# ada-shen/Interpret_quality

Hardware: AMD Instinct MI355X
Metric: coalitions/sec (masked forward passes/sec), PointNet 1024-pt ModelNet10 (higher is better)
Workload: dtype f32; 1 GPU; PointNet ModelNet10-style Shapley, 32 regions x 1000 permutations per cloud (33000 coalitions per step per GPU), BASELINE configs[1]; permutations sampled and masked on the device inside the timed step; num_points=1024, num_regions=32, permutations=1000, parallelism=clouds sharded over 1 GPU(s), one all_gather_into_tensor of the logits per step

## Files before the change

include/iq.h:

```cpp
#ifndef IQ_H_
#define IQ_H_

#include <stddef.h>
#include <stdint.h>

#ifdef __cplusplus
extern "C" {
#endif

typedef void* iq_stream_t;

enum {
    IQ_OK = 0,
    IQ_EINVAL = -1,
    IQ_ELAUNCH = -2,
    IQ_EWORKSPACE = -3,
    IQ_EUNSUPPORTED = -4
};

#define IQ_MAX_REGIONS 64
#define IQ_MAX_POINTS 4096
#define IQ_NUM_FEAT 1024
#define IQ_MAX_EXACT_PLAYERS 24
#define IQ_MAX_WIDE_REGIONS 1024

#define IQ_ABI_VERSION 111
int iq_version(void);
const char* iq_last_error(void);


int iq_mask_shapley(const float* cloud , const int32_t* region_id ,
                    const int32_t* orders , const float* center , float* out,
                    int N, int R, int bs, int channel_first, iq_stream_t stream);

int iq_mask_interaction(const float* cloud , const int32_t* region_id ,
                        const int32_t* pairs , const uint64_t* ctx_mask ,
                        const float* center , float* out ,
                        int N, int R, int nb, iq_stream_t stream);

int iq_mask_coalitions(const float* cloud , const int32_t* region_id ,
                       const uint64_t* keep , const float* center , float* out,
                       int N, int B, int channel_first, iq_stream_t stream);

int iq_check_index_range(const int32_t* idx, size_t count, int lo, int hi, uint32_t* scratch ,
                         iq_stream_t stream);


int iq_sample_permutations(uint32_t* mt_state , int32_t* orders , int S, int R, iq_stream_t stream);

size_t iq_sample_workspace_bytes(int S, int R);
int iq_sample_permutations_ws(uint32_t* mt_state , int32_t* orders , int S, int R, void* workspace,
                              size_t workspace_bytes, iq_stream_t stream);

int iq_prefix_keep_masks(const int32_t* orders , uint64_t* keep , int S, int R, iq_stream_t stream);

int iq_context_keep_masks(const int32_t* pairs , const int32_t* contexts , uint64_t* keep ,
                          int P, int C, int m, iq_stream_t stream);


int iq_reward(const float* logits , int label, int modified, float* v ,
              int B, int C, iq_stream_t stream);

int iq_shapley_accum(const float* v , const int32_t* orders ,
                     double* sv_rows, double* phi_sum, const int32_t* snap_counts, int n_snap,
                     double* snaps, int R, int S, iq_stream_t stream);

int iq_interaction_reduce(const float* v , float* out , int n, iq_stream_t stream);


int iq_region_assign(const float* cloud , const int32_t* fps_idx ,
                     int32_t* region_id , int N, int R, iq_stream_t stream);

int iq_fps(const float* xyz, int32_t* idx, int B, int N, int S, iq_stream_t stream);

typedef struct iq_smoothness_params {
    double step;
    double enum_step;
    double var_threshold;
    double dist_threshold;
// ... 234 lines not shown
```

include/iq_debug.h:

```cpp
#ifndef IQ_DEBUG_H_
#define IQ_DEBUG_H_

#include "iq.h"

#ifdef __cplusplus
extern "C" {
#endif

int iq_profile_enable(int on);
int iq_profile_read_work(int slot, double* total_ms, int* launches, double* total_work);
int iq_set_tuning(int key, int value);
int iq_profile_read(int slot, double* total_ms, int* launches);

int iq_debug_mfma_sustained(double seconds, float* scratch , size_t scratch_floats, double* tflops ,
                            double* clock_ghz , iq_stream_t stream);
int iq_debug_mfma_sustained_shape(int shape, double seconds, float* scratch , size_t scratch_floats, double* tflops ,
                                  double* clock_ghz , iq_stream_t stream);

#ifdef __cplusplus
}
#endif
#endif
```

interpret_quality_amd/_lib.py:

```python
import ctypes
import os

from . import build as _build

_HERE = os.path.dirname(os.path.abspath(__file__))

c_f32p = ctypes.c_void_p
c_ptr = ctypes.c_void_p


class IqError(RuntimeError):
    pass


class DenseLayer(ctypes.Structure):
    _fields_ = [("w", ctypes.c_void_p), ("b", ctypes.c_void_p), ("cin", ctypes.c_int32), ("cout", ctypes.c_int32),
                ("w_bf3", ctypes.c_void_p)]


class PointNetWeights(ctypes.Structure):
    _fields_ = [
        ("stn_in", ctypes.c_void_p),
        ("stn_c2", DenseLayer), ("stn_c3", DenseLayer), ("stn_fc1", DenseLayer), ("stn_fc2", DenseLayer),
        ("stn_fc3", DenseLayer),
# ... 78 lines not shown
                                    _I, _I, _I, _I, _I, _P]),
    "iq_pointnet_coalitions_crt": (_I, [ctypes.POINTER(PointNetWeights), _P, _P, _P, _P, _P, _P, _P, _P, _P, _SZ,
                                        _I, _I, _I, _I, _I, _P]),
    "iq_pointnet_flops_per_coalition": (ctypes.c_double, [_I]),
    "iq_ball_query": (_I, [_P, _P, ctypes.c_float, _I, _P, _I, _I, _I, _P]),
    "iq_pointnet2_workspace_bytes": (_SZ, [_I]),
    "iq_pointnet2_forward": (_I, [ctypes.POINTER(PointNet2Weights), _P, _P, _P, _SZ, _I, _I, _P]),
    "iq_pointnet2_coalitions_workspace_bytes": (_SZ, [_I, _I, _I]),
    "iq_pointnet2_coalitions": (_I, [ctypes.POINTER(PointNet2Weights), _P, _P, _P, _P, _P, _P, _P, _SZ, _I, _I, _I, _P]),
    "iq_knn": (_I, [_P, _P, _P, _SZ, _I, _I, _I, _I, _P]),
    "iq_dgcnn_workspace_bytes": (_SZ, [_I, _I]),
    "iq_dgcnn_forward": (_I, [ctypes.POINTER(DgcnnWeights), _P, _P, _P, _SZ, _I, _I, _I, _P]),
    "iq_dgcnn_coalitions": (_I, [ctypes.POINTER(DgcnnWeights), _P, _P, _P, _P, _P, _P, _P, _SZ, _I, _I, _I, _I, _P]),
    "iq_pointconv_workspace_bytes": (_SZ, [_I, _I]),
    "iq_pointconv_forward": (_I, [ctypes.POINTER(PointConvWeights), _P, _P, _P, _SZ, _I, _I, _P]),
    "iq_pointconv_coalitions_workspace_bytes": (_SZ, [_I, _I, _I]),
    "iq_pointconv_coalitions": (_I, [ctypes.POINTER(PointConvWeights), _P, _P, _P, _P, _P, _P, _P, _SZ, _I, _I, _I, _P]),
    "iq_pointconv_tables_bytes": (_SZ, [_I, _I]),
    "iq_pointconv_coalitions_cached": (_I, [ctypes.POINTER(PointConvWeights), _P, _P, _P, _P, _P, _P, _P, _SZ, _I, _I, _I,
                                          ctypes.POINTER(ctypes.c_int), _P]),
    "iq_index_points": (_I, [_P, _P, _P, _I, _I, _I, _I, _P]),
    "iq_group_points": (_I, [_P, _P, _P, _P, _P, _I, _I, _I, _I, _I, _I, _P]),
    "iq_edgeconv_gather": (_I, [_P, _P, _P, _I, _I, _I, _I, _I, _P]),
    "iq_knn_point": (_I, [_P, _P, _I, _P, _P, _SZ, _I, _I, _I, _P]),
    "iq_sort_neighbours": (_I, [_P, _P, _P, _I, _I, _I, _I, _I, _P]),
    "iq_density": (_I, [_P, ctypes.c_double, _P, _I, _I, _P]),
    "iq_enum_keep_masks": (_I, [_P, ctypes.c_uint64, _SZ, _P, _I, ctypes.c_uint64, _P]),
    "iq_exact_scratch_bytes": (_SZ, [_I, _I]),
    "iq_exact_shapley": (_I, [_P, _I, _P, _P, _SZ, _P]),
    "iq_exact_interactions": (_I, [_P, _I, _P, _I, _P, _P, _SZ, _P]),
    "iq_moebius": (_I, [_P, _I, _P, _P]),
    "iq_prefix_keep_masks_wide": (_I, [_P, _P, _I, _I, _P]),
    "iq_context_keep_masks_wide": (_I, [_P, _P, _P, _I, _I, _I, _I, _P]),
    "iq_mask_coalitions_wide": (_I, [_P, _P, _P, _P, _P, _I, _I, _I, _I, _P]),
    "iq_region_assign_wide": (_I, [_P, _P, _P, _I, _I, _P]),
    "iq_shapley_accum_wide": (_I, [_P, _P, _P, _P, _P, _I, _P, _I, _I, _P]),
    "iq_pointnet_wide_workspace_bytes": (_SZ, [_I, _I, _I, _I]),
    "iq_pointnet_coalitions_wide": (_I, [ctypes.POINTER(PointNetWeights), _P, _P, _P, _P, _P, _P, _P, _P, _SZ,
                                         _I, _I, _I, _I, _I, _P]),
    "iq_pointnet_prefix_coalitions_wide": (_I, [ctypes.POINTER(PointNetWeights), _P, _P, _P, _P, _P, _P, _P, _P, _SZ,
                                                _I, _I, _I, _I, _P]),
    "iq_dgcnn_coalitions_wide": (_I, [ctypes.POINTER(DgcnnWeights), _P, _P, _P, _P, _P, _P, _P, _SZ, _I, _I, _I, _I, _I, _P]),
    "iq_pointnet2_coalitions_wide": (_I, [ctypes.POINTER(PointNet2Weights), _P, _P, _P, _P, _P, _P, _P, _SZ, _I, _I, _I, _I, _P]),
    "iq_pointconv_coalitions_wide": (_I, [ctypes.POINTER(PointConvWeights), _P, _P, _P, _P, _P, _P, _P, _SZ, _I, _I, _I, _I, _P]),
    "iq_pointconv_coalitions_cached_wide": (_I, [ctypes.POINTER(PointConvWeights), _P, _P, _P, _P, _P, _P, _P, _SZ, _I, _I, _I,
                                               ctypes.POINTER(ctypes.c_int), _I, _P]),
    "iq_profile_enable": (_I, [_I]),
    "iq_set_tuning": (_I, [_I, _I]),
    "iq_profile_read_work": (_I, [_I, ctypes.POINTER(ctypes.c_double), ctypes.POINTER(ctypes.c_int), ctypes.POINTER(ctypes.c_double)]),
    "iq_profile_read": (_I, [_I, ctypes.POINTER(ctypes.c_double), ctypes.POINTER(ctypes.c_int)]),
    "iq_debug_mfma_sustained": (_I, [ctypes.c_double, _P, _SZ, ctypes.POINTER(ctypes.c_double), ctypes.POINTER(ctypes.c_double), _P]),
    "iq_debug_mfma_sustained_shape": (_I, [_I, ctypes.c_double, _P, _SZ, ctypes.POINTER(ctypes.c_double),
                                           ctypes.POINTER(ctypes.c_double), _P]),
}

_lib = None
ABI_VERSION = 111


def lib_path():
    return os.environ.get("IQ_LIBPATH") or _build.LIBPATH


def load():
    global _lib
    if _lib is not None:
        return _lib
    import torch
    path = lib_path()
    if not os.path.exists(path):
        raise IqError("libiq_hip.so not found at %s - run `python -m interpret_quality_amd.build` "
                      "(there is no CPU or PyTorch fallback for the HIP path)" % path)
    lib = ctypes.CDLL(path)
    for name, (res, args) in SIGNATURES.items():
        fn = getattr(lib, name)
        fn.restype = res
        fn.argtypes = args
    if lib.iq_version() != ABI_VERSION:
        raise IqError("%s reports ABI version %d, these bindings are written for %d - rebuild it (python -m interpret_quality_amd.build "
                      "--force)" % (path, lib.iq_version(), ABI_VERSION))
    _lib = lib
    return lib


def check(rc, what):
    if rc != 0:
        msg = load().iq_last_error()
        raise IqError("%s failed (%d): %s" % (what, rc, msg.decode() if msg else ""))
```

interpret_quality_amd/csrc/iq_pointnet.hip:

```cpp
#include <algorithm>

#include "iq_pointnet_chain.h"

namespace {

template <int MAXR>
__device__ __forceinline__ void pn_prepare_body(const int32_t* __restrict__ region_id, uint16_t* __restrict__ sorted_pts,
                                                int32_t* __restrict__ roff, int N, int R) {
    constexpr int kWaves = kThreads / 64;
    __shared__ int16_t rid[kMaxN];
    __shared__ int cnt[kWaves][MAXR + 1];
    const int cloud = blockIdx.x, tid = threadIdx.x, wave = tid >> 6, lane = tid & 63;
    for (int r = tid; r <= R; r += kThreads)
        for (int w = 0; w < kWaves; ++w) cnt[w][r] = 0;
    for (int p = tid; p < N; p += kThreads) {
        const int r = region_id[(size_t)cloud * N + p];
        rid[p] = (int16_t)((unsigned)r < (unsigned)R ? r : R);
    }
    __syncthreads();
    const int per = (N + kThreads - 1) / kThreads * 64;
    const int begin = min(wave * per, N), end = min(begin + per, N);
    for (int p = begin + lane; p < end; p += 64) atomicAdd(&cnt[wave][rid[p]], 1);
    __syncthreads();
    if (wave == 0) {
// ... 317 lines not shown
    const int item = blockIdx.x * blockDim.x + threadIdx.x;
    int bin = 0, pos = 0;
    if (item < B) {
        bin = bin_of[item];
        pos = atomicAdd(&lh[bin], 1);
    }
    __syncthreads();
    if (threadIdx.x < kBins && lh[threadIdx.x]) base[threadIdx.x] = atomicAdd(&cursor[threadIdx.x], lh[threadIdx.x]);
    __syncthreads();
    if (item < B) order[base[bin] + pos] = item;
}

constexpr int kOrderThreads = 1024, kOrderPer = 4, kOrderFusedMax = kOrderThreads * kOrderPer;

__global__ __launch_bounds__(kOrderThreads) void pn_order_fused_kernel(const int32_t* __restrict__ nrows_all,
                                                                       int32_t* __restrict__ order, int B) {
    __shared__ int lh[kBins];
    const int tid = threadIdx.x, lane = tid & 63;
    if (tid < kBins) lh[tid] = 0;
    __syncthreads();
    int bin[kOrderPer], pos[kOrderPer];
#pragma unroll
    for (int j = 0; j < kOrderPer; ++j) {
        const int item = tid + j * kOrderThreads;
        if (item < B) {
            const int rows = nrows_all[item] & 0xffff;
            bin[j] = kBins - 1 - min(kBins - 1, (rows + kMC - 1) / kMC);
            pos[j] = atomicAdd(&lh[bin[j]], 1);
        }
    }
    __syncthreads();
    if (tid < 64) {
        int carry = 0;
        for (int b0 = 0; b0 < kBins; b0 += 64) {
            const int b = b0 + lane, c = b < kBins ? lh[b] : 0;
            int inc = c;
#pragma unroll
            for (int off = 1; off < 64; off <<= 1) {
                const int t = __shfl_up(inc, off);
                if (lane >= off) inc += t;
            }
            if (b < kBins) lh[b] = carry + inc - c;
            carry += __shfl(inc, 63);
        }
    }
    __syncthreads();
#pragma unroll
    for (int j = 0; j < kOrderPer; ++j) {
        const int item = tid + j * kOrderThreads;
        if (item < B) order[lh[bin[j]] + pos[j]] = item;
    }
}

constexpr int kDupRepOff = kBins;
static_assert(iq::align_up((kBins + 2) * sizeof(int32_t), 256) == iq::align_up(kBins * sizeof(int32_t), 256), "room behind hist");

__global__ __launch_bounds__(kOrderThreads) void pn_dup_rep_kernel(const int32_t* __restrict__ nrows_all, int32_t* __restrict__ rep,
                                                                   int B, int N) {
    __shared__ int first[2];
    if (threadIdx.x < 2) first[threadIdx.x] = B;
    __syncthreads();
    for (int item = threadIdx.x; item < B; item += kOrderThreads) {
        const int kind = dup_kind(nrows_all[item], N);
        if (kind >= 0) atomicMin(&first[kind], item);
    }
    __syncthreads();
    if (threadIdx.x < 2) rep[threadIdx.x] = first[threadIdx.x];
}

__global__ __launch_bounds__(kThreads) void pn_dup_copy_kernel(const int32_t* __restrict__ nrows_all, const int32_t* __restrict__ rep,
                                                               float* __restrict__ out, int32_t* __restrict__ argrow, int N) {
    const int item = blockIdx.x;
    const int kind = dup_kind(nrows_all[item], N);
    if (kind < 0) return;
    const int src = rep[kind];
    if (src == item) return;
    static_assert(kFeat == 4 * kThreads, "one float4 per thread");
    reinterpret_cast<f32x4*>(out + (size_t)item * kFeat)[threadIdx.x] = reinterpret_cast<const f32x4*>(out + (size_t)src * kFeat)[threadIdx.x];
    if (argrow) {
        const int4 v = reinterpret_cast<const int4*>(argrow + (size_t)src * kFeat)[threadIdx.x];
        reinterpret_cast<int4*>(argrow + (size_t)item * kFeat)[threadIdx.x] = v;
    }
}

__global__ __launch_bounds__(kThreads) void pn_stn_gather_kernel(const float* __restrict__ G,
                                                                 const int32_t* __restrict__ nrows_all,
                                                                 const uint64_t* __restrict__ keep,
                                                                 const int32_t* __restrict__ cloud_of,
                                                                 float* __restrict__ out, int R, int nclouds,
                                                                 int with_centre) {
    const int item = blockIdx.x;
    const int cloud = cloud_of ? cloud_of[item] : (nclouds == 1 ? 0 : item);
    const uint64_t full = R >= 64 ? ~0ull : ((1ull << R) - 1);
    const uint64_t k = (keep ? keep[item] : ~0ull) & full;
    const int per = R + with_centre;
    const f32x4* g4 = reinterpret_cast<const f32x4*>(G) + (size_t)cloud * per * (kFeat / 4) + threadIdx.x;
    f32x4 m = {-INFINITY, -INFINITY, -INFINITY, -INFINITY};
    for (int r = 0; r < R; ++r) {
        if ((k >> r) & 1) {
            const f32x4 v = g4[(size_t)r * (kFeat / 4)];
            m[0] = fmaxf(m[0], v[0]); m[1] = fmaxf(m[1], v[1]); m[2] = fmaxf(m[2], v[2]); m[3] = fmaxf(m[3], v[3]);
        }
    }
    if (nrows_all[item] >> 16) {
        const f32x4 v = g4[(size_t)R * (kFeat / 4)];
        m[0] = fmaxf(m[0], v[0]); m[1] = fmaxf(m[1], v[1]); m[2] = fmaxf(m[2], v[2]); m[3] = fmaxf(m[3], v[3]);
    }
    reinterpret_cast<f32x4*>(out)[(size_t)item * (kFeat / 4) + threadIdx.x] = m;
}

__global__ __launch_bounds__(kThreads) void pn_stn_gather_wide_kernel(const float* __restrict__ G,
                                                                      const int32_t* __restrict__ nrows_all,
                                                                      const uint64_t* __restrict__ keep,
                                                                      const int32_t* __restrict__ cloud_of,
                                                                      float* __restrict__ out, int R, int W, int nclouds,
                                                                      int with_centre) {
    __shared__ uint64_t ks[kMaxW];
    const int item = blockIdx.x;
    const int cloud = cloud_of ? cloud_of[item] : (nclouds == 1 ? 0 : item);
    if ((int)threadIdx.x < W) {
        uint64_t k = keep ? keep[(size_t)item * W + threadIdx.x] : ~0ull;
        if ((int)threadIdx.x == W - 1 && (R & 63)) k &= (1ull << (R & 63)) - 1;
        ks[threadIdx.x] = k;
    }
    __syncthreads();
    const int per = R + with_centre;
    const f32x4* g4 = reinterpret_cast<const f32x4*>(G) + (size_t)cloud * per * (kFeat / 4) + threadIdx.x;
    f32x4 m = {-INFINITY, -INFINITY, -INFINITY, -INFINITY};
// ... 64 lines not shown
            if (i > R) break;
            f32x4 w = m;
            if (flag_s[i]) { w[0] = fmaxf(w[0], c[0]); w[1] = fmaxf(w[1], c[1]); w[2] = fmaxf(w[2], c[2]); w[3] = fmaxf(w[3], c[3]); }
            o4[(size_t)i * (kFeat / 4)] = w;
            m[0] = fmaxf(m[0], v[q][0]); m[1] = fmaxf(m[1], v[q][1]); m[2] = fmaxf(m[2], v[q][2]); m[3] = fmaxf(m[3], v[q][3]);
        }
    }
}

__global__ __launch_bounds__(kThreads) void pn_fill_rows_kernel(float* __restrict__ out, const float* __restrict__ image, int B) {
    const size_t t = (size_t)blockIdx.x * kThreads + threadIdx.x;
    if (t >= (size_t)B * 1024) return;
    reinterpret_cast<f32x4*>(out)[t] = reinterpret_cast<const f32x4*>(image)[t & 1023];
}

using iq::launch_linear;

struct Workspace {
    uint16_t* sorted_pts;
    int32_t* roff;
    uint16_t* rows_pre;
    int32_t* nrows_pre;
    uint16_t* rows;
    int32_t* nrows;
    int32_t* order;
    int32_t* bin_of;
    int32_t* hist;
    float* G;
    float* gbuf;
    float* h1;
    float* h2;
    float* trans;
    float* tfp;
    uint16_t* fc3_bf3;
    size_t bytes;
};

Workspace carve(void* base, int B, int nclouds, int N, int R, int roff_entries = IQ_MAX_REGIONS + 1) {
    Workspace w;
    size_t off = 0;
    auto take = [&](size_t bytes) {
        size_t o = off;
        off = iq::align_up(off + bytes, 256);
        return reinterpret_cast<char*>(base) + o;
    };
    w.sorted_pts = reinterpret_cast<uint16_t*>(take((size_t)nclouds * N * sizeof(uint16_t)));
    w.roff = reinterpret_cast<int32_t*>(take((size_t)nclouds * roff_entries * sizeof(int32_t)));
    w.rows_pre = reinterpret_cast<uint16_t*>(take((size_t)nclouds * (R + 1) * kRowCap * sizeof(uint16_t)));
    w.nrows_pre = reinterpret_cast<int32_t*>(take((size_t)nclouds * (R + 1) * sizeof(int32_t)));
    w.rows = reinterpret_cast<uint16_t*>(take((size_t)B * kRowCap * sizeof(uint16_t)));
    w.nrows = reinterpret_cast<int32_t*>(take((size_t)B * sizeof(int32_t)));
    w.order = reinterpret_cast<int32_t*>(take((size_t)B * sizeof(int32_t)));
    w.bin_of = reinterpret_cast<int32_t*>(take((size_t)B * sizeof(int32_t)));
    w.hist = reinterpret_cast<int32_t*>(take((size_t)(kBins + 2) * sizeof(int32_t)));
    w.G = reinterpret_cast<float*>(take((size_t)nclouds * (R + 1) * kFeat * sizeof(float)));
    w.gbuf = reinterpret_cast<float*>(take((size_t)B * kFeat * sizeof(float)));
    w.h1 = reinterpret_cast<float*>(take((size_t)B * 512 * sizeof(float)));
    w.h2 = reinterpret_cast<float*>(take((size_t)B * 256 * sizeof(float)));
    w.trans = reinterpret_cast<float*>(take((size_t)B * 9 * sizeof(float)));
    w.tfp = reinterpret_cast<float*>(take((size_t)B * 4096 * sizeof(float)));
    w.fc3_bf3 = reinterpret_cast<uint16_t*>(take(iq_packed_bf3_elems(4096, 256) * sizeof(uint16_t)));
    w.bytes = off;
    return w;
}

}

extern "C" size_t iq_pointnet_workspace_bytes(int B, int nclouds, int N, int R) {
    if (B < 0 || nclouds < 0 || N < 0 || R < 0) return 0;
    return carve(nullptr, B, nclouds, N, R).bytes;
}

extern "C" double iq_pointnet_flops_per_coalition(int N) {
    const double per_point = 426377.0;
    const double fc = 3.0 * (1024.0 * 512 + 512.0 * 256) + 256.0 * (9 + 4096 + 10);
    return 2.0 * (per_point * N + fc);
}

extern "C" int iq_pointnet_coalitions(const iq_pointnet_weights* w, const float* clouds, const float* centers,
                                      const int32_t* region_id, const uint64_t* keep, const int32_t* cloud_of,
                                      float* logits, float* trans_feat_packed, void* workspace,
                                      size_t workspace_bytes, int B, int nclouds, int N, int R,
                                      int channel_first, iq_stream_t stream) {
    return iq_pointnet_coalitions_crt(w, clouds, centers, region_id, keep, cloud_of, logits, trans_feat_packed, nullptr, workspace,
                                      workspace_bytes, B, nclouds, N, R, channel_first, stream);
}

namespace {

int pointnet_coalitions(const iq_pointnet_weights* w, const float* clouds, const float* centers, const int32_t* region_id,
                        const uint64_t* keep, int wide_words, const int32_t* orders, const int32_t* cloud_of, float* logits,
                        float* trans_feat_packed, int32_t* crt_points, void* workspace, size_t workspace_bytes, int B, int nclouds,
                        int N, int R, int channel_first, iq_stream_t stream) {
    const char* who = orders ? "iq_pointnet_prefix_coalitions_wide"
                             : wide_words ? "iq_pointnet_coalitions_wide" : "iq_pointnet_coalitions";
    IQ_REQUIRE(B >= 0 && nclouds >= 1, "%s: B=%d nclouds=%d", who, B, nclouds);
    IQ_REQUIRE(w && clouds && region_id && (logits || B == 0), "%s: null pointer", who);
    IQ_REQUIRE(N >= 1 && N <= kMaxN, "%s: N=%d not in [1,%d]", who, N, kMaxN);
    const int max_regions = wide_words ? IQ_MAX_WIDE_REGIONS : IQ_MAX_REGIONS;
    IQ_REQUIRE(R >= 1 && R <= max_regions, "%s: R=%d not in [1,%d]", who, R, max_regions);
    const int groups = orders ? B / (R + 1) : B;
    IQ_REQUIRE(cloud_of || nclouds == 1 || nclouds == groups, "%s: cloud_of required when 1 < nclouds != %s", who, orders ? "S" : "B");
    const int with_centre = centers ? 1 : 0;
    IQ_REQUIRE(centers || !(keep || orders), "%s: %s need centers", who, orders ? "prefix coalitions" : "keep masks");
    if (B == 0) return IQ_OK;
    const size_t need = wide_words ? iq_pointnet_wide_workspace_bytes(B, nclouds, N, R) : iq_pointnet_workspace_bytes(B, nclouds, N, R);
    if (!workspace || workspace_bytes < need)
        return iq::fail(IQ_EWORKSPACE, "%s: workspace %zu < %zu bytes", who, workspace_bytes, need);
    Workspace ws = wide_words ? carve(workspace, B, nclouds, N, R, R + 1) : carve(workspace, B, nclouds, N, R);
    hipStream_t st = iq::as_stream(stream);
    int rc;
    iq::ProfileSpan call_span(iq::kSlotCall, st);

    const int pre_items = nclouds * (R + with_centre);
    const int32_t* item_cloud = orders ? (nclouds > 1 ? ws.bin_of : nullptr) : cloud_of;
    if (wide_words) {
        hipLaunchKernelGGL(pn_prepare_wide_kernel, dim3(nclouds), dim3(kThreads), 0, st, region_id, ws.sorted_pts, ws.roff, N, R);
        if ((rc = iq::check_launch("pn_prepare_wide_kernel"))) return rc;
        hipLaunchKernelGGL(pn_rows_wide_kernel, dim3(pre_items), dim3(64), 0, st, ws.sorted_pts, ws.roff, nullptr, nullptr,
                           ws.rows_pre, ws.nrows_pre, N, R, wide_words, nclouds, with_centre, 1);
        if ((rc = iq::check_launch("pn_rows_wide_kernel"))) return rc;
        if (orders) {
            hipLaunchKernelGGL(pn_rows_prefix_kernel, dim3(groups), dim3(kThreads), 0, st, ws.sorted_pts, ws.roff, orders, cloud_of,
                               ws.rows, ws.nrows, N, R, nclouds, with_centre);
            if ((rc = iq::check_launch("pn_rows_prefix_kernel"))) return rc;
        } else {
            hipLaunchKernelGGL(pn_rows_wide_kernel, dim3(B), dim3(64), 0, st, ws.sorted_pts, ws.roff, keep, cloud_of, ws.rows,
                               ws.nrows, N, R, wide_words, nclouds, with_centre, 0);
            if ((rc = iq::check_launch("pn_rows_wide_kernel"))) return rc;
        }
    } else {
        hipLaunchKernelGGL(pn_prepare_kernel, dim3(nclouds), dim3(kThreads), 0, st, region_id, ws.sorted_pts, ws.roff, N, R);
        if ((rc = iq::check_launch("pn_prepare_kernel"))) return rc;
        hipLaunchKernelGGL(pn_rows_kernel, dim3(pre_items), dim3(64), 0, st, ws.sorted_pts, ws.roff, nullptr, nullptr,
                           ws.rows_pre, ws.nrows_pre, N, R, nclouds, with_centre, 1);
        hipLaunchKernelGGL(pn_rows_kernel, dim3(B), dim3(64), 0, st, ws.sorted_pts, ws.roff, keep, cloud_of, ws.rows,
                           ws.nrows, N, R, nclouds, with_centre, 0);
        if ((rc = iq::check_launch("pn_rows_kernel"))) return rc;
    }
    if (B <= kOrderFusedMax) {
        hipLaunchKernelGGL(pn_order_fused_kernel, dim3(1), dim3(kOrderThreads), 0, st, ws.nrows, ws.order, B);
    } else {
        if (hipMemsetAsync(ws.hist, 0, kBins * sizeof(int32_t), st) != hipSuccess)
            return iq::fail(IQ_ELAUNCH, "%s: memset failed", who);
        hipLaunchKernelGGL(pn_order_count_kernel, dim3((B + kThreads - 1) / kThreads), dim3(kThreads), 0, st, ws.nrows,
                           ws.bin_of, ws.hist, B);
        hipLaunchKernelGGL(pn_order_scan_kernel, dim3(1), dim3(64), 0, st, ws.hist);
        hipLaunchKernelGGL(pn_order_scatter_kernel, dim3((B + kThreads - 1) / kThreads), dim3(kThreads), 0, st,
                           ws.bin_of, ws.hist, ws.order, B);
    }
    if ((rc = iq::check_launch("pn_order kernels"))) return rc;
    const int32_t* dup_rep = nullptr;
    if (nclouds == 1 && !wide_words && B > 1 && iq::twin() != iq::kTwinChainNoDedup) {
        hipLaunchKernelGGL(pn_dup_rep_kernel, dim3(1), dim3(kOrderThreads), 0, st, ws.nrows, ws.hist + kDupRepOff, B, N);
        if ((rc = iq::check_launch("pn_dup_rep_kernel"))) return rc;
        dup_rep = ws.hist + kDupRepOff;
    }

    ChainArgs a{};
    a.clouds = clouds;
    if (channel_first) { a.ps = 1; a.cs = N; } else { a.ps = 3; a.cs = 1; }
    a.cl = 3 * N;
    a.centers = centers;
    a.rows = ws.rows_pre;
    a.nrows = ws.nrows_pre;
    a.item_order = nullptr;
    a.N = N; a.R = R; a.nclouds = nclouds; a.with_centre = with_centre;
    a.tail16 = iq::twin() != iq::kTwinChainL3Fp32NoTail16;
    a.l3_single = iq::twin() == iq::kTwinChainL3Single;


    a.cloud_of = nullptr; a.trans = nullptr;
    a.w_in = w->stn_in;
    a.w1 = nullptr; a.b1 = nullptr;
    a.w2 = w->stn_c2.w; a.b2 = w->stn_c2.b;
    a.w3 = w->stn_c3.w; a.b3 = w->stn_c3.b;
    a.out = ws.G;
    a.items = pre_items;
    {
        iq::ProfileSpan span(iq::kSlotPrepool, st);
        launch_chain<kPrepool>(a, st);
    }
    if ((rc = iq::check_launch("pn_chain_kernel<prepool>"))) return rc;

    if (orders)
        hipLaunchKernelGGL(pn_stn_prefix_kernel, dim3(groups, kFeat / 256), dim3(64), 0, st, ws.G, ws.nrows, orders, cloud_of, ws.gbuf,
                           item_cloud ? ws.bin_of : nullptr, R, nclouds, with_centre);
    else if (wide_words)
        hipLaunchKernelGGL(pn_stn_gather_wide_kernel, dim3(B), dim3(kThreads), 0, st, ws.G, ws.nrows, keep, cloud_of, ws.gbuf,
                           R, wide_words, nclouds, with_centre);
    else
        hipLaunchKernelGGL(pn_stn_gather_kernel, dim3(B), dim3(kThreads), 0, st, ws.G, ws.nrows, keep, cloud_of, ws.gbuf,
                           R, nclouds, with_centre);
    if ((rc = iq::check_launch(orders ? "pn_stn_prefix_kernel" : wide_words ? "pn_stn_gather_wide_kernel" : "pn_stn_gather_kernel")))
        return rc;
    if ((rc = launch_linear(ws.gbuf, kFeat, w->stn_fc1, ws.h1, 512, B, 1, st, nullptr, nullptr, 0, true))) return rc;
    if ((rc = launch_linear(ws.h1, 512, w->stn_fc2, ws.h2, 256, B, 1, st, nullptr, nullptr, 0, true))) return rc;
    if ((rc = launch_linear(ws.h2, 256, w->stn_fc3, ws.trans, 9, B, 0, st, nullptr, nullptr, 0, true))) return rc;

    a.cloud_of = item_cloud; a.trans = ws.trans;
    a.rows = ws.rows; a.nrows = ws.nrows;
    a.item_order = ws.order;
    a.dup_rep = dup_rep;
    a.w_in = w->feat_in;
    a.items = B;
    a.out = ws.gbuf;
    float* tfp = trans_feat_packed ? trans_feat_packed : ws.tfp;
    if (w->fstn_c1.w) {
        a.w1 = w->fstn_c1.w; a.b1 = w->fstn_c1.b;
        a.w2 = w->fstn_c2.w; a.b2 = w->fstn_c2.b;
        a.w3 = w->fstn_c3.w; a.b3 = w->fstn_c3.b; a.w3_bf3 = reinterpret_cast<const unsigned short*>(w->fstn_c3_bf3);
        a.w2_bf3 = reinterpret_cast<const unsigned short*>(w->fstn_c2_bf3);
        {
            iq::ProfileSpan span(iq::kSlotFstn, st);
            launch_chain<kFstn>(a, st);
        }
        if (dup_rep) hipLaunchKernelGGL(pn_dup_copy_kernel, dim3(B), dim3(kThreads), 0, st, ws.nrows, dup_rep, ws.gbuf, nullptr, N);
        if ((rc = iq::check_launch("pn_chain_kernel<fstn>"))) return rc;
        if ((rc = launch_linear(ws.gbuf, kFeat, w->fstn_fc1, ws.h1, 512, B, 1, st, nullptr, nullptr, 0, true))) return rc;
        if ((rc = launch_linear(ws.h1, 512, w->fstn_fc2, ws.h2, 256, B, 1, st, nullptr, nullptr, 0, true))) return rc;
        iq_dense_layer fc3 = w->fstn_fc3;
        IQ_REQUIRE(fc3.cin == 256 && fc3.cout == 4096, "%s: fstn_fc3 is %d -> %d, not 256 -> 4096", who, fc3.cin, fc3.cout);
        if (!fc3.w_bf3 && iq::twin() != iq::kTwinDenseFp32) {
            if ((rc = iq::launch_split_bf3(fc3.w, ws.fc3_bf3, 4096, 256, st))) return rc;
            fc3.w_bf3 = ws.fc3_bf3;
        }
        if ((rc = launch_linear(ws.h2, 256, fc3, tfp, 4096, B, 0, st, nullptr, nullptr, 0, true))) return rc;
    } else {
        IQ_REQUIRE(w->fstn_fc3.b, "%s: without a feature STN, fstn_fc3.b must hold the packed identity", who);
        hipLaunchKernelGGL(pn_fill_rows_kernel, dim3((unsigned)(((size_t)B * 1024 + kThreads - 1) / kThreads)), dim3(kThreads), 0, st,
                           tfp, w->fstn_fc3.b, B);
        if ((rc = iq::check_launch("pn_fill_rows_kernel"))) return rc;
    }

    a.argrow = crt_points;
    a.w1 = tfp; a.b1 = nullptr;
    a.w2 = w->feat_c2.w; a.b2 = w->feat_c2.b;
    a.w3 = w->feat_c3.w; a.b3 = w->feat_c3.b; a.w3_bf3 = reinterpret_cast<const unsigned short*>(w->feat_c3_bf3);
    a.w2_bf3 = reinterpret_cast<const unsigned short*>(w->feat_c2_bf3);
    {
        iq::ProfileSpan span(iq::kSlotTrunk, st);
        launch_chain<kTrunk>(a, st);
    }
    if (dup_rep) hipLaunchKernelGGL(pn_dup_copy_kernel, dim3(B), dim3(kThreads), 0, st, ws.nrows, dup_rep, ws.gbuf, crt_points, N);
    if ((rc = iq::check_launch("pn_chain_kernel<trunk>"))) return rc;
    if ((rc = launch_linear(ws.gbuf, kFeat, w->cls_fc1, ws.h1, 512, B, 1, st, nullptr, nullptr, 0, true))) return rc;
    if ((rc = launch_linear(ws.h1, 512, w->cls_fc2, ws.h2, 256, B, 1, st, nullptr, nullptr, 0, true))) return rc;
    if ((rc = launch_linear(ws.h2, 256, w->cls_fc3, logits, w->cls_fc3.cout, B, 0, st, nullptr, nullptr, 0, true))) return rc;
    return IQ_OK;
}

}

extern "C" int iq_pointnet_coalitions_crt(const iq_pointnet_weights* w, const float* clouds, const float* centers,
                                          const int32_t* region_id, const uint64_t* keep, const int32_t* cloud_of,
                                          float* logits, float* trans_feat_packed, int32_t* crt_points, void* workspace,
                                          size_t workspace_bytes, int B, int nclouds, int N, int R,
                                          int channel_first, iq_stream_t stream) {
    return pointnet_coalitions(w, clouds, centers, region_id, keep, 0, nullptr, cloud_of, logits, trans_feat_packed, crt_points, workspace,
                               workspace_bytes, B, nclouds, N, R, channel_first, stream);
}

extern "C" size_t iq_pointnet_wide_workspace_bytes(int B, int nclouds, int N, int R) {
    if (B < 0 || nclouds < 0 || N < 0 || R < 0) return 0;
    return carve(nullptr, B, nclouds, N, R, R + 1).bytes;
}

extern "C" int iq_pointnet_coalitions_wide(const iq_pointnet_weights* w, const float* clouds, const float* centers,
                                           const int32_t* region_id, const uint64_t* keep, const int32_t* cloud_of,
                                           float* logits, float* trans_feat_packed, void* workspace, size_t workspace_bytes,
                                           int B, int nclouds, int N, int R, int channel_first, iq_stream_t stream) {
    IQ_REQUIRE(R >= 1 && R <= IQ_MAX_WIDE_REGIONS, "iq_pointnet_coalitions_wide: R=%d not in [1,%d]", R, IQ_MAX_WIDE_REGIONS);
    return pointnet_coalitions(w, clouds, centers, region_id, keep, (R + 63) / 64, nullptr, cloud_of, logits, trans_feat_packed,
                               nullptr, workspace, workspace_bytes, B, nclouds, N, R, channel_first, stream);
}

extern "C" int iq_pointnet_prefix_coalitions_wide(const iq_pointnet_weights* w, const float* clouds, const float* centers,
                                                  const int32_t* region_id, const int32_t* orders, const int32_t* cloud_of,
                                                  float* logits, float* trans_feat_packed, void* workspace, size_t workspace_bytes,
                                                  int S, int nclouds, int N, int R, iq_stream_t stream) {
    IQ_REQUIRE(R >= 1 && R <= IQ_MAX_WIDE_REGIONS, "iq_pointnet_prefix_coalitions_wide: R=%d not in [1,%d]", R, IQ_MAX_WIDE_REGIONS);
    IQ_REQUIRE(S >= 0 && S <= 0x7fffffff / (R + 1), "iq_pointnet_prefix_coalitions_wide: S=%d (R=%d)", S, R);
    IQ_REQUIRE(centers && (orders || S == 0), "iq_pointnet_prefix_coalitions_wide: null pointer");
    return pointnet_coalitions(w, clouds, centers, region_id, nullptr, (R + 63) / 64, orders, cloud_of, logits, trans_feat_packed,
                               nullptr, workspace, workspace_bytes, S * (R + 1), nclouds, N, R, 0, stream);
}

extern "C" int iq_pack_fstn_fc3(const float* w, const float* b, float* out_w, float* out_b, int32_t* perm) {
    IQ_REQUIRE(w && b && out_w && out_b, "iq_pack_fstn_fc3: null pointer");
    float* tmp = new float[4096 * 256];
    for (int nt = 0; nt < 2; ++nt)
        for (int kb = 0; kb < 8; ++kb)
            for (int lane = 0; lane < 64; ++lane)
                for (int j = 0; j < 4; ++j) {
                    const int n = nt * 32 + (lane & 31), k = 8 * kb + 4 * (lane >> 5) + j;
                    const int e = ((nt * 8 + kb) * 64 + lane) * 4 + j;
                    const int src = k * 64 + n;
                    for (int c = 0; c < 256; ++c) tmp[(size_t)e * 256 + c] = w[(size_t)src * 256 + c];
                    out_b[e] = b[src] + (k == n ? 1.f : 0.f);
                    if (perm) perm[e] = src;
                }
    const int rc = iq_pack_weight(tmp, out_w, 4096, 256);
    delete[] tmp;
    return rc;
}
```

interpret_quality_amd/csrc/iq_pointnet_chain.h:

```cpp
#pragma once
#include <type_traits>

#include "iq_common.h"
#include "iq_profile.h"

#include "iq_bf3.h"
#include "iq_mfma.h"

namespace {

constexpr int kFeat = IQ_NUM_FEAT;
constexpr int kMC = 64;
constexpr int kMC96 = 96;
constexpr int kMaxN = 4096;
constexpr int kThreads = 256;
constexpr int kRowCap = kMaxN + kMC;

enum ChainMode { kPrepool = 0, kFstn = 1, kTrunk = 2, kFstn64 = 3, kTrunk64 = 4 };

constexpr int kLd1 = 64 + 4;
constexpr int kLd2 = 128 + 4;

struct ChainArgs {
    const float* clouds;
// ... 259 lines not shown
template <int ROWS, int PLANEB>
__device__ __forceinline__ void stage0b_planes(unsigned char* act0, const float* xs, const f32x4 (&wi)[4], int t) {
    const int cq = t & 15;
#pragma unroll
    for (int i = 0; i < ROWS / 16; ++i) {
        const int row = (t >> 4) + 16 * i;
        const f32x4 xv = *reinterpret_cast<const f32x4*>(xs + row * 4);
        f32x4 v;
#pragma unroll
        for (int j = 0; j < 4; ++j) v[j] = fmaxf(fmaf(wi[j][2], xv[2], fmaf(wi[j][1], xv[1], wi[j][0] * xv[0])) + wi[j][3], 0.f);
        row4_to_planes<PLANEB>(act0 + row * kLd1B + 16 * ((cq >> 1) ^ swz_of_row<kLd1B>(row)) + 8 * (cq & 1), v);
    }
}

struct L1Raw { f32x4 r[2][2]; };
__device__ __forceinline__ L1Raw l1_raw_load(const __amdgpu_buffer_rsrc_t& rs, int ln, int wave_s) {
    const int voff = ((ln >> 4) * 64 + 16 * (wave_s & 1) + (ln & 15)) * 16;
    L1Raw w;
#pragma unroll
    for (int t = 0; t < 2; ++t)
#pragma unroll
        for (int h = 0; h < 2; ++h)
            w.r[t][h] = __builtin_bit_cast(f32x4, __builtin_amdgcn_raw_buffer_load_b128(rs, voff + 512 * h, ((wave_s >> 1) * 8 + 4 * t) * kFragBytes, 0));
    return w;
}
template <int MT, int PLANEB, bool RELU>
__device__ __forceinline__ void l1_bf3(const unsigned char* act0, unsigned char* act1, const L1Raw& raw, f32x4 bq, int ln, int wave_s) {
    constexpr int G = MT % 3 == 0 ? 3 : 2;
    static_assert(MT % G == 0, "m-tiles go G at a time");
    const int a0off = a16_lane_off<kLd1B>(ln), l15 = ln & 15;
    const B3 w[2] = {b3_split8(raw.r[0][0], raw.r[0][1]), b3_split8(raw.r[1][0], raw.r[1][1])};
#pragma unroll
    for (int p = 0; p < MT; p += G) {
        f32x4 acc[G];
#pragma unroll
        for (int i = 0; i < G; ++i) acc[i] = (f32x4){0.f, 0.f, 0.f, 0.f};
#pragma unroll
        for (int t = 0; t < 2; ++t) {
            bf16x8 af[G][3];
#pragma unroll
            for (int i = 0; i < G; ++i) a16_load<kLd1B, PLANEB>(af[i], act0, a0off, p + i, t);
            mfma16_bf3_col_tr<G>(w[t], af, acc);
        }
#pragma unroll
        for (int i = 0; i < G; ++i) {
            f32x4 v = acc[i];
            if (RELU) v = bias_relu4(v, bq);
            c16_tile_to_planes_swz<kLd1B, PLANEB>(act1, 16 * (p + i) + l15, 2 * wave_s, ln, v);
        }
        __builtin_amdgcn_sched_barrier(0);
    }
}

__device__ __forceinline__ int dup_kind(int nrows_word, int N) { return nrows_word == N ? 0 : nrows_word == ((1 << 16) | 1) ? 1 : -1; }

__device__ __forceinline__ __amdgpu_buffer_rsrc_t chain_rsrc(const void* base) {
    return __builtin_amdgcn_make_buffer_rsrc(const_cast<void*>(base), 0, 0x7fffffff, 0x00020000);
}

template <int MODE, int MC>
struct PointFetcher {
    const ChainArgs& a;
    const int item, cloud, nchunks, frow;
    const bool fetcher;
    const uint16_t* rowp;
    float px = 0.f, py = 0.f, pz = 0.f;
    int pnext = 0;

    __device__ __forceinline__ PointFetcher(const ChainArgs& a_, int item_, int cloud_, int nchunks_, int lane, int wave)
        : a(a_), item(item_), cloud(cloud_), nchunks(nchunks_), frow(wave * (MC / 4) + lane), fetcher(lane < MC / 4),
          rowp(a_.rows + (size_t)item_ * kRowCap + frow) {
        if (fetcher) {
            load_point(rowp[0]);
            if (nchunks > 1) pnext = rowp[MC];
        }
    }
    __device__ __forceinline__ void load_point(int p) {
        if (p == a.N) {
            px = a.centers[cloud * 3]; py = a.centers[cloud * 3 + 1]; pz = a.centers[cloud * 3 + 2];
        } else {
            const float* src = a.clouds + (size_t)cloud * a.cl + (size_t)p * a.ps;
            px = src[0]; py = src[a.cs]; pz = src[2 * a.cs];
        }
    }
    __device__ __forceinline__ void stage0a(float* xs) const {
        if (fetcher) {
            float x = px, y = py, z = pz;
            if (MODE != kPrepool) {
                const float* t9 = a.trans + (size_t)item * 9;
                const float x2 = fmaf(z, t9[6], fmaf(y, t9[3], x * t9[0]));
                const float y2 = fmaf(z, t9[7], fmaf(y, t9[4], x * t9[1]));
                const float z2 = fmaf(z, t9[8], fmaf(y, t9[5], x * t9[2]));
                x = x2; y = y2; z = z2;
            }
            *reinterpret_cast<f32x4*>(xs + frow * 4) = (f32x4){x, y, z, 0.f};
        }
    }
    __device__ __forceinline__ void advance(int ch) {
        if (fetcher && ch + 1 < nchunks) {
            load_point(pnext);
            if (ch + 2 < nchunks) pnext = rowp[(ch + 2) * MC];
        }
    }
};

template <int PLANEB>
__device__ __forceinline__ void l2_store_bf3(unsigned char* act2, const f32x4 (&acc)[2], f32x4 bq, int row, int c, int ln) {
#pragma unroll
// ... 284 lines not shown
#pragma unroll
            for (int f = 0; f < 4; ++f) bw[f] = b3_load16_l2(w2rs, boff, wave_s, f >> 1, f & 1);
            f32x4 acc[2][3][2];
#pragma unroll
            for (int hf = 0; hf < 2; ++hf)
#pragma unroll
                for (int mt = 0; mt < 3; ++mt) { acc[hf][mt][0] = (f32x4){0.f, 0.f, 0.f, 0.f}; acc[hf][mt][1] = acc[hf][mt][0]; }
            __syncthreads();
#pragma unroll
            for (int t = 0; t < 2; ++t) {
#pragma unroll
                for (int mt = 0; mt < 3; ++mt) {
                    if (mt < mts) {
                        bf16x8 af[2][3];
#pragma unroll
                        for (int pi = 0; pi < 2; ++pi) a16_load<kLd1B, kPlane96_1>(af[pi], act1, a1off, 2 * mt + pi, t);
#pragma unroll
                        for (int hf = 0; hf < 2; ++hf) mfma16_bf3_col_tr<2>(bw[2 * t + hf], af, acc[hf][mt]);
                    }
                    __builtin_amdgcn_sched_barrier(0);
                }
            }
            __syncthreads();
#pragma unroll
            for (int hf = 0; hf < 2; ++hf) {
                const int c = wave_s * 32 + 16 * hf;
                const f32x4 bq = *reinterpret_cast<const f32x4*>(a.b2 + c + 4 * kq);
#pragma unroll
                for (int mt = 0; mt < 3; ++mt)
                    if (mt < mts) l2_store_bf3<kPlane96>(img, acc[hf][mt], bq, mt * 32 + l15, c, ln);
            }
        }
        __syncthreads();
        l3_pass_bf3_2x2<mts, kPlane96>(w3rs, b16_lane_off(ln), img, a16_lane_off<kLdB>(ln), wave_s, runmax, ring3);
    };
    for (int ch = 0; ch + 1 < nchunks; ++ch) chunk(std::integral_constant<int, 3>{}, ch);
    const int rows_last = nrows - (nchunks - 1) * kMC96;
    if (rows_last > 64)      chunk(std::integral_constant<int, 3>{}, nchunks - 1);
    else if (rows_last > 32) chunk(std::integral_constant<int, 2>{}, nchunks - 1);
    else                     chunk(std::integral_constant<int, 1>{}, nchunks - 1);
    chain_epilogue_bf3<MODE, false>(a, item, wave, lane, runmax, nullptr);
}

template <int CM, int L3V, bool ARGMAX = false>
__global__ __launch_bounds__(kThreads, L3V == 3 ? 2 : 3) void pn_chain_kernel(ChainArgs a) {
    constexpr int MODE = CM >= kFstn64 ? CM - kFstn64 + kFstn : CM;
    static_assert(CM < kFstn64 || (L3V == 3 && !ARGMAX), "kFstn64 / kTrunk64: the 64-row twins of the product instantiations only");
    const int item = a.item_order ? a.item_order[blockIdx.x] : blockIdx.x;
    int cloud;
    if (MODE == kPrepool) cloud = item / (a.R + a.with_centre);
    else cloud = a.cloud_of ? a.cloud_of[item] : (a.nclouds == 1 ? 0 : item);

    const int nrows = a.nrows[item] & 0xffff;
    if (MODE != kPrepool && a.dup_rep) {
        const int kind = dup_kind(a.nrows[item], a.N);
        if (kind >= 0 && a.dup_rep[kind] != item) return;
    }
    if (nrows == 0) {
        float* outp = a.out + (size_t)item * kFeat;
        for (int c = threadIdx.x; c < kFeat; c += kThreads) outp[c] = -INFINITY;
        return;
    }
    if constexpr (L3V == 2) chain_fp32<MODE, ARGMAX>(a, item, cloud, nrows);
    else if constexpr ((CM == kFstn || CM == kTrunk) && !ARGMAX) chain_bf3_96<MODE>(a, item, cloud, nrows);
    else chain_bf3_64<MODE, ARGMAX>(a, item, cloud, nrows);
}

template <int MODE>
void launch_chain(const ChainArgs& a, hipStream_t st) {
    const bool fp32_l3 = iq::twin() == iq::kTwinChainL3Fp32 || iq::twin() == iq::kTwinChainL3Fp32NoTail16;
    const bool bf3 = a.w3_bf3 && a.w2_bf3 && !fp32_l3;
    if constexpr (MODE == kTrunk) {
        if (a.argrow) {
            if (bf3) hipLaunchKernelGGL((pn_chain_kernel<kTrunk, 3, true>), dim3(a.items), dim3(kThreads), 0, st, a);
            else     hipLaunchKernelGGL((pn_chain_kernel<kTrunk, 2, true>), dim3(a.items), dim3(kThreads), 0, st, a);
            return;
        }
    }
    if constexpr (MODE != kPrepool) {
        if (bf3) {
            if (a.l3_single) hipLaunchKernelGGL((pn_chain_kernel<MODE - kFstn + kFstn64, 3>), dim3(a.items), dim3(kThreads), 0, st, a);
            else             hipLaunchKernelGGL((pn_chain_kernel<MODE, 3>), dim3(a.items), dim3(kThreads), 0, st, a);
            return;
        }
    }
    hipLaunchKernelGGL((pn_chain_kernel<MODE, 2>), dim3(a.items), dim3(kThreads), 0, st, a);
}

}
```

interpret_quality_amd/hip_ops.py:

```python
import ctypes

import numpy as np
import torch

from . import _lib


def _stream():
    return ctypes.c_void_p(torch.cuda.current_stream().cuda_stream)


def _dev(t, dtype, name):
    if not isinstance(t, torch.Tensor) or not t.is_cuda:
        raise _lib.IqError("%s must be a CUDA/HIP tensor (the HIP path has no CPU fallback)" % name)
    if t.dtype != dtype:
        raise _lib.IqError("%s must be %s, got %s" % (name, dtype, t.dtype))
    if not t.is_contiguous():
        raise _lib.IqError("%s must be contiguous" % name)
    return ctypes.c_void_p(t.data_ptr())


def _p(t):
    return ctypes.c_void_p(t.data_ptr()) if t is not None else ctypes.c_void_p(0)

# ... 489 lines not shown


SMOOTHNESS_MODES = ("linearity", "planarity", "scattering")


def smoothness_enum(cloud, region_id, num_regions, mode, objective, step=1e-3, enum_step=0.05, var_threshold=0.003,
                    dist_threshold=0.03, stop_ratio=0.5, epochs=50, max_iteration=100, origin=None, project_to_bound=False,
                    entry="iq_smoothness_enum"):
    lib = _lib.load()
    n, r, e = cloud.shape[0], int(num_regions), int(epochs)
    dev = cloud.device
    out = {"data": torch.empty((e, n, 3), dtype=torch.float32, device=dev),
           "smoothness": torch.empty((e, r), dtype=torch.float32, device=dev),
           "var": torch.empty((e, r, 3), dtype=torch.float32, device=dev),
           "orig": torch.empty((r, 4), dtype=torch.float32, device=dev),
           "stop_epoch": torch.empty((r,), dtype=torch.int32, device=dev)}
    prm = _lib.SmoothnessParams(step, enum_step, var_threshold, dist_threshold, stop_ratio, e, int(max_iteration), int(bool(project_to_bound)), 0)
    if mode not in SMOOTHNESS_MODES or objective not in ("inc", "dec"):
        raise _lib.IqError("smoothness_enum: mode %r / objective %r" % (mode, objective))
    org = _dev(origin, torch.float32, "origin") if origin is not None else ctypes.c_void_p(0)
    _lib.check(getattr(lib, entry)(_dev(cloud, torch.float32, "cloud"), org, _dev(region_id, torch.int32, "region_id"), n, r,
                                   SMOOTHNESS_MODES.index(mode), 1 if objective == "inc" else -1, ctypes.byref(prm),
                                   _p(out["data"]), _p(out["smoothness"]), _p(out["var"]), _p(out["orig"]),
                                   _p(out["stop_epoch"]), _stream()), entry)
    return out


MAX_SMOOTHNESS_POINTS = 1024


def smoothness_enum_wide(cloud, region_id, num_regions, mode, objective, **kw):
    wide_words(num_regions)
    if not 1 <= cloud.shape[0] <= MAX_SMOOTHNESS_POINTS:
        raise _lib.IqError("smoothness_enum_wide: N=%d points, the enumeration takes 1 .. %d" % (cloud.shape[0], MAX_SMOOTHNESS_POINTS))
    return smoothness_enum(cloud, region_id, num_regions, mode, objective, entry="iq_smoothness_enum_wide", **kw)


class PackedLinear:

    def __init__(self, weight, bias, device, bf3=False):
        from .engine import Packer
        self.cout, self.cin = np.shape(weight)
        self._packer = Packer(device)
        self.struct = self._packer.dense(np.asarray(weight), bias, bf3=bf3)


def linear(x, layer, act=0):
    lib = _lib.load()
    m = x.shape[0]
    out = torch.empty((m, layer.cout), dtype=torch.float32, device=x.device)
    _lib.check(lib.iq_linear(_dev(x, torch.float32, "x"), x.shape[1], ctypes.byref(layer.struct), _p(out), layer.cout, m, int(act),
                             _stream()), "iq_linear")
    return out
```

Measured before the change: 1.000 million coalitions/s.

## Generalize PointNet coalition dedup to hash-table over full keep masks

Replaces the old duplicate detection, which caught only the full and empty coalitions of a single cloud, with a GPU open-addressing hash table keyed on (keep mask, cloud). Every item maps to the smallest-index item with the same mask, and only those representatives run the chain kernels. Results are then copied to the duplicates. With 1000 random permutations over 32 regions, small and large prefixes repeat often, so more forward passes can be skipped, at the cost of a memset and two small kernels per step plus a wider copy kernel launch.

```diff
diff --git a/include/iq.h b/include/iq.h
--- a/include/iq.h
+++ b/include/iq.h
@@ -24,7 +24,7 @@
 #define IQ_MAX_EXACT_PLAYERS 24
 #define IQ_MAX_WIDE_REGIONS 1024
 
-#define IQ_ABI_VERSION 111
+#define IQ_ABI_VERSION 112
 int iq_version(void);
 const char* iq_last_error(void);
 
diff --git a/include/iq_debug.h b/include/iq_debug.h
--- a/include/iq_debug.h
+++ b/include/iq_debug.h
@@ -17,6 +17,9 @@
 int iq_debug_mfma_sustained_shape(int shape, double seconds, float* scratch , size_t scratch_floats, double* tflops ,
                                   double* clock_ghz , iq_stream_t stream);
 
+int iq_debug_pointnet_reps(const uint64_t* keep , const int32_t* cloud_of , int B, int nclouds, int R,
+                           int32_t* rep_out , void* scratch , size_t scratch_bytes, iq_stream_t stream);
+
 #ifdef __cplusplus
 }
 #endif
diff --git a/interpret_quality_amd/_lib.py b/interpret_quality_amd/_lib.py
--- a/interpret_quality_amd/_lib.py
+++ b/interpret_quality_amd/_lib.py
@@ -154,10 +154,11 @@
     "iq_debug_mfma_sustained": (_I, [ctypes.c_double, _P, _SZ, ctypes.POINTER(ctypes.c_double), ctypes.POINTER(ctypes.c_double), _P]),
     "iq_debug_mfma_sustained_shape": (_I, [_I, ctypes.c_double, _P, _SZ, ctypes.POINTER(ctypes.c_double),
                                            ctypes.POINTER(ctypes.c_double), _P]),
+    "iq_debug_pointnet_reps": (_I, [_P, _P, _I, _I, _I, _P, _P, _SZ, _P]),
 }
 
 _lib = None
-ABI_VERSION = 111
+ABI_VERSION = 112
 
 
 def lib_path():
diff --git a/interpret_quality_amd/csrc/iq_pointnet.hip b/interpret_quality_amd/csrc/iq_pointnet.hip
--- a/interpret_quality_amd/csrc/iq_pointnet.hip
+++ b/interpret_quality_amd/csrc/iq_pointnet.hip
@@ -393,28 +393,74 @@
     }
 }
 
-constexpr int kDupRepOff = kBins;
-static_assert(iq::align_up((kBins + 2) * sizeof(int32_t), 256) == iq::align_up(kBins * sizeof(int32_t), 256), "room behind hist");
-
-__global__ __launch_bounds__(kOrderThreads) void pn_dup_rep_kernel(const int32_t* __restrict__ nrows_all, int32_t* __restrict__ rep,
-                                                                   int B, int N) {
-    __shared__ int first[2];
-    if (threadIdx.x < 2) first[threadIdx.x] = B;
-    __syncthreads();
-    for (int item = threadIdx.x; item < B; item += kOrderThreads) {
-        const int kind = dup_kind(nrows_all[item], N);
-        if (kind >= 0) atomicMin(&first[kind], item);
-    }
-    __syncthreads();
-    if (threadIdx.x < 2) rep[threadIdx.x] = first[threadIdx.x];
-}
-
-__global__ __launch_bounds__(kThreads) void pn_dup_copy_kernel(const int32_t* __restrict__ nrows_all, const int32_t* __restrict__ rep,
-                                                               float* __restrict__ out, int32_t* __restrict__ argrow, int N) {
+__host__ __device__ inline size_t rep_slots(int B) {
+    size_t s = 4;
+    while (s < 2 * (size_t)B) s <<= 1;
+    return s;
+}
+
+__device__ __forceinline__ uint32_t rep_hash(uint64_t k, int cloud) {
+    uint64_t x = k * 0x9E3779B97F4A7C15ull + (uint64_t)(uint32_t)cloud * 0xC2B2AE3D27D4EB4Full;
+    x ^= x >> 29;
+    x *= 0xBF58476D1CE4E5B9ull;
+    return (uint32_t)(x >> 32);
+}
+
+__global__ __launch_bounds__(kThreads) void pn_rep_insert_kernel(const uint64_t* __restrict__ keep, const int32_t* __restrict__ cloud_of,
+                                                                 int32_t* table, int32_t* __restrict__ rep, int B, int R,
+                                                                 uint32_t slot_mask) {
+    const int item = blockIdx.x * kThreads + threadIdx.x, lane = threadIdx.x & 63;
+    const bool live = item < B;
+    const uint64_t full = R >= 64 ? ~0ull : ((1ull << R) - 1);
+    const uint64_t k = live ? keep[item] & full : 0;
+    const int cloud = live && cloud_of ? cloud_of[item] : 0;
+    const int k_lo = (int)(uint32_t)k, k_hi = (int)(uint32_t)(k >> 32);
+    int leader = lane;
+    for (uint64_t todo = __ballot(live); todo;) {
+        const int l = __ffsll((unsigned long long)todo) - 1;
+        const bool same = live && k_lo == __builtin_amdgcn_readlane(k_lo, l) && k_hi == __builtin_amdgcn_readlane(k_hi, l) &&
+                          cloud == __builtin_amdgcn_readlane(cloud, l);
+        if (same) leader = l;
+        todo &= ~__ballot(same);
+    }
+    int slot = 0;
+    if (live && leader == lane) {
+        uint32_t h = rep_hash(k, cloud) & slot_mask;
+        for (;;) {
+            int old = __atomic_load_n(&table[h], __ATOMIC_RELAXED);
+            if (old == -1) old = atomicCAS(&table[h], -1, item);
+            if (old == -1) break;
+            if ((keep[old] & full) == k && (cloud_of ? cloud_of[old] : 0) == cloud) {
+                if (item < old) atomicMin(&table[h], item);
+                break;
+            }
+            h = (h + 1) & slot_mask;
+        }
+        slot = (int)h;
+    }
+    slot = __shfl(slot, leader);
+    if (live) rep[item] = slot;
+}
+
+__global__ __launch_bounds__(kThreads) void pn_rep_write_kernel(const int32_t* __restrict__ table, int32_t* __restrict__ rep, int B) {
+    const int item = blockIdx.x * kThreads + threadIdx.x;
+    if (item < B) rep[item] = table[rep[item]];
+}
+
+int launch_reps(const uint64_t* keep, const int32_t* cloud_of, int B, int R, int32_t* rep, int32_t* table, hipStream_t st) {
+    const size_t slots = rep_slots(B);
+    if (hipMemsetAsync(table, 0xff, slots * sizeof(int32_t), st) != hipSuccess)
+        return iq::fail(IQ_ELAUNCH, "pn_rep kernels: memset failed");
+    const dim3 grid((B + kThreads - 1) / kThreads);
+    hipLaunchKernelGGL(pn_rep_insert_kernel, grid, dim3(kThreads), 0, st, keep, cloud_of, table, rep, B, R, (uint32_t)(slots - 1));
+    hipLaunchKernelGGL(pn_rep_write_kernel, grid, dim3(kThreads), 0, st, table, rep, B);
+    return iq::check_launch("pn_rep kernels");
+}
+
+__global__ __launch_bounds__(kThreads) void pn_dup_copy_kernel(const int32_t* __restrict__ rep, float* __restrict__ out,
+                                                               int32_t* __restrict__ argrow) {
     const int item = blockIdx.x;
-    const int kind = dup_kind(nrows_all[item], N);
-    if (kind < 0) return;
-    const int src = rep[kind];
+    const int src = rep[item];
     if (src == item) return;
     static_assert(kFeat == 4 * kThreads, "one float4 per thread");
     reinterpret_cast<f32x4*>(out + (size_t)item * kFeat)[threadIdx.x] = reinterpret_cast<const f32x4*>(out + (size_t)src * kFeat)[threadIdx.x];
@@ -585,7 +631,7 @@
     w.nrows = reinterpret_cast<int32_t*>(take((size_t)B * sizeof(int32_t)));
     w.order = reinterpret_cast<int32_t*>(take((size_t)B * sizeof(int32_t)));
     w.bin_of = reinterpret_cast<int32_t*>(take((size_t)B * sizeof(int32_t)));
-    w.hist = reinterpret_cast<int32_t*>(take((size_t)(kBins + 2) * sizeof(int32_t)));
+    w.hist = reinterpret_cast<int32_t*>(take((size_t)kBins * sizeof(int32_t)));
     w.G = reinterpret_cast<float*>(take((size_t)nclouds * (R + 1) * kFeat * sizeof(float)));
     w.gbuf = reinterpret_cast<float*>(take((size_t)B * kFeat * sizeof(float)));
     w.h1 = reinterpret_cast<float*>(take((size_t)B * 512 * sizeof(float)));
@@ -684,10 +730,10 @@
     }
     if ((rc = iq::check_launch("pn_order kernels"))) return rc;
     const int32_t* dup_rep = nullptr;
-    if (nclouds == 1 && !wide_words && B > 1 && iq::twin() != iq::kTwinChainNoDedup) {
-        hipLaunchKernelGGL(pn_dup_rep_kernel, dim3(1), dim3(kOrderThreads), 0, st, ws.nrows, ws.hist + kDupRepOff, B, N);
-        if ((rc = iq::check_launch("pn_dup_rep_kernel"))) return rc;
-        dup_rep = ws.hist + kDupRepOff;
+    if (!wide_words && !orders && keep && B > 1 && (cloud_of || nclouds == 1) && iq::twin() != iq::kTwinChainNoDedup) {
+        static_assert(sizeof(int32_t) * 4 <= sizeof(float) * 512, "rep_slots(B) < 4 B int32 inside h1's (B,512) floats");
+        if ((rc = launch_reps(keep, cloud_of, B, R, ws.bin_of, reinterpret_cast<int32_t*>(ws.h1), st))) return rc;
+        dup_rep = ws.bin_of;
     }
 
     ChainArgs a{};
@@ -748,7 +794,7 @@
             iq::ProfileSpan span(iq::kSlotFstn, st);
             launch_chain<kFstn>(a, st);
         }
-        if (dup_rep) hipLaunchKernelGGL(pn_dup_copy_kernel, dim3(B), dim3(kThreads), 0, st, ws.nrows, dup_rep, ws.gbuf, nullptr, N);
+        if (dup_rep) hipLaunchKernelGGL(pn_dup_copy_kernel, dim3(B), dim3(kThreads), 0, st, dup_rep, ws.gbuf, nullptr);
         if ((rc = iq::check_launch("pn_chain_kernel<fstn>"))) return rc;
         if ((rc = launch_linear(ws.gbuf, kFeat, w->fstn_fc1, ws.h1, 512, B, 1, st, nullptr, nullptr, 0, true))) return rc;
         if ((rc = launch_linear(ws.h1, 512, w->fstn_fc2, ws.h2, 256, B, 1, st, nullptr, nullptr, 0, true))) return rc;
@@ -775,7 +821,7 @@
         iq::ProfileSpan span(iq::kSlotTrunk, st);
         launch_chain<kTrunk>(a, st);
     }
-    if (dup_rep) hipLaunchKernelGGL(pn_dup_copy_kernel, dim3(B), dim3(kThreads), 0, st, ws.nrows, dup_rep, ws.gbuf, crt_points, N);
+    if (dup_rep) hipLaunchKernelGGL(pn_dup_copy_kernel, dim3(B), dim3(kThreads), 0, st, dup_rep, ws.gbuf, crt_points);
     if ((rc = iq::check_launch("pn_chain_kernel<trunk>"))) return rc;
     if ((rc = launch_linear(ws.gbuf, kFeat, w->cls_fc1, ws.h1, 512, B, 1, st, nullptr, nullptr, 0, true))) return rc;
     if ((rc = launch_linear(ws.h1, 512, w->cls_fc2, ws.h2, 256, B, 1, st, nullptr, nullptr, 0, true))) return rc;
@@ -792,6 +838,19 @@
                                           int channel_first, iq_stream_t stream) {
     return pointnet_coalitions(w, clouds, centers, region_id, keep, 0, nullptr, cloud_of, logits, trans_feat_packed, crt_points, workspace,
                                workspace_bytes, B, nclouds, N, R, channel_first, stream);
+}
+
+extern "C" int iq_debug_pointnet_reps(const uint64_t* keep, const int32_t* cloud_of, int B, int nclouds, int R, int32_t* rep_out,
+                                      void* scratch, size_t scratch_bytes, iq_stream_t stream) {
+    IQ_REQUIRE(B >= 0 && nclouds >= 1, "iq_debug_pointnet_reps: B=%d nclouds=%d", B, nclouds);
+    IQ_REQUIRE(R >= 1 && R <= IQ_MAX_REGIONS, "iq_debug_pointnet_reps: R=%d not in [1,%d]", R, IQ_MAX_REGIONS);
+    IQ_REQUIRE(cloud_of || nclouds == 1, "iq_debug_pointnet_reps: cloud_of required when nclouds > 1");
+    if (B == 0) return IQ_OK;
+    IQ_REQUIRE(keep && rep_out, "iq_debug_pointnet_reps: null pointer");
+    const size_t need = rep_slots(B) * sizeof(int32_t);
+    if (!scratch || scratch_bytes < need)
+        return iq::fail(IQ_EWORKSPACE, "iq_debug_pointnet_reps: scratch %zu < %zu bytes", scratch_bytes, need);
+    return launch_reps(keep, cloud_of, B, R, rep_out, reinterpret_cast<int32_t*>(scratch), iq::as_stream(stream));
 }
 
 extern "C" size_t iq_pointnet_wide_workspace_bytes(int B, int nclouds, int N, int R) {
diff --git a/interpret_quality_amd/csrc/iq_pointnet_chain.h b/interpret_quality_amd/csrc/iq_pointnet_chain.h
--- a/interpret_quality_amd/csrc/iq_pointnet_chain.h
+++ b/interpret_quality_amd/csrc/iq_pointnet_chain.h
@@ -335,8 +335,6 @@
     }
 }
 
-__device__ __forceinline__ int dup_kind(int nrows_word, int N) { return nrows_word == N ? 0 : nrows_word == ((1 << 16) | 1) ? 1 : -1; }
-
 __device__ __forceinline__ __amdgpu_buffer_rsrc_t chain_rsrc(const void* base) {
     return __builtin_amdgcn_make_buffer_rsrc(const_cast<void*>(base), 0, 0x7fffffff, 0x00020000);
 }
@@ -727,10 +725,7 @@
     else cloud = a.cloud_of ? a.cloud_of[item] : (a.nclouds == 1 ? 0 : item);
 
     const int nrows = a.nrows[item] & 0xffff;
-    if (MODE != kPrepool && a.dup_rep) {
-        const int kind = dup_kind(a.nrows[item], a.N);
-        if (kind >= 0 && a.dup_rep[kind] != item) return;
-    }
+    if (MODE != kPrepool && a.dup_rep && a.dup_rep[item] != item) return;
     if (nrows == 0) {
         float* outp = a.out + (size_t)item * kFeat;
         for (int c = threadIdx.x; c < kFeat; c += kThreads) outp[c] = -INFINITY;
diff --git a/interpret_quality_amd/hip_ops.py b/interpret_quality_amd/hip_ops.py
--- a/interpret_quality_amd/hip_ops.py
+++ b/interpret_quality_amd/hip_ops.py
@@ -565,3 +565,15 @@
     _lib.check(lib.iq_linear(_dev(x, torch.float32, "x"), x.shape[1], ctypes.byref(layer.struct), _p(out), layer.cout, m, int(act),
                              _stream()), "iq_linear")
     return out
+
+
+def pointnet_reps(keep, cloud_of=None, num_regions=64, nclouds=1, scratch_bytes=None):
+    lib = _lib.load()
+    b = keep.shape[0]
+    rep = torch.empty((b,), dtype=torch.int32, device=keep.device)
+    nbytes = 16 * max(b, 1) if scratch_bytes is None else int(scratch_bytes)
+    scratch = torch.empty((max(nbytes, 1),), dtype=torch.uint8, device=keep.device)
+    _lib.check(lib.iq_debug_pointnet_reps(_dev(keep, torch.int64, "keep"), _dev(cloud_of, torch.int32, "cloud_of") if cloud_of is not None
+                                          else ctypes.c_void_p(0), b, int(nclouds), int(num_regions), _p(rep), _p(scratch), nbytes,
+                                          _stream()), "iq_debug_pointnet_reps")
+    return rep
```

Result: faster. 1.115 million coalitions/s, median of 6 (+11.4%).
